# eliesgalvira/pragma-dsp

Measured on AMD Instinct MI355X. Metric: batched 1D FFT GSample/s at N=4096 batch=65536; achieved HBM GB/s vs peak, higher is better.
Workload: dtype f32

## Files before the change

### pragma-dsp_amd/csrc/pdsp_fft_kernel.h

```cpp
#pragma once

#include <hip/hip_runtime.h>

#include <type_traits>
#include <utility>

#include "pdsp_radix.h"

namespace pdsp {

#ifdef PDSP_STAMPS
__device__ unsigned long long pdsp_stamp_acc[64];
#define PDSP_STAMP_INIT() unsigned long long stamp_last_ = clock64()
#define PDSP_STAMP(slot)                                                          \
  do {                                                                            \
    __builtin_amdgcn_sched_barrier(0);                                            \
    const unsigned long long t_ = clock64();                                      \
    if (threadIdx.x == 0) atomicAdd(&pdsp_stamp_acc[slot], t_ - stamp_last_);     \
    stamp_last_ = clock64();                                                      \
    __builtin_amdgcn_sched_barrier(0);                                            \
  } while (0)
#else
#define PDSP_STAMP_INIT() ((void)0)
#define PDSP_STAMP(slot) ((void)0)
#endif

template <typename T> struct vec2;
template <> struct vec2<float> { using type = float2; };
template <> struct vec2<double> { using type = double2; };

template <typename T>
using cx = T __attribute__((ext_vector_type(2)));

template <int... Is, class F>
__device__ __forceinline__ void static_for_impl(std::integer_sequence<int, Is...>, F &&f) {
  (f(std::integral_constant<int, Is>{}), ...);
}
template <int N, class F>
__device__ __forceinline__ void static_for(F &&f) {
  static_for_impl(std::make_integer_sequence<int, N>{}, static_cast<F &&>(f));
}

constexpr int ilog2(int v) {
  int l = 0;
  while ((1 << l) < v) ++l;
  return l;
}
constexpr int bitrev(int x, int bits) {
  int y = 0;
  for (int b = 0; b < bits; ++b) {
    y = (y << 1) | (x & 1);
    x >>= 1;
  }
  return y;
}

template <typename T, int E, int I = 0>
__device__ __forceinline__ void pin_regs(T __attribute__((ext_vector_type(2))) (&a)[E]) {
  if constexpr (I < E) {
    asm volatile("" : "+v"(a[I]));
    pin_regs<T, E, I + 1>(a);
  }
}


template <typename T>
__device__ __forceinline__ cx<T> mul_neg_i(const cx<T> a) {
  return cx<T>{a.y, -a.x};
}
template <typename T>
__device__ __forceinline__ cx<T> conj(const cx<T> a) {
  return cx<T>{a.x, -a.y};
}
template <typename T>
__device__ __forceinline__ cx<T> add_mul_neg_i(const cx<T> a, const cx<T> b) {
  if constexpr (std::is_same_v<T, float>) {
    return __builtin_elementwise_fma(__builtin_shufflevector(b, b, 1, 0), cx<float>{1.0f, -1.0f}, a);
  } else {
    return cx<T>{a.x + b.y, a.y - b.x};
  }
}
template <typename T>
__device__ __forceinline__ cx<T> add_mul_pos_i(const cx<T> a, const cx<T> b) {
  if constexpr (std::is_same_v<T, float>) {
    return __builtin_elementwise_fma(__builtin_shufflevector(b, b, 1, 0), cx<float>{-1.0f, 1.0f}, a);
  } else {
    return cx<T>{a.x - b.y, a.y + b.x};
  }
}
template <typename T>
__device__ __forceinline__ cx<T> cmul(const cx<T> a, const cx<T> w) {
  if constexpr (std::is_same_v<T, float>) {
    cx<float> r;
    asm("v_pk_mul_f32 %0, %1, %2 op_sel:[0,0] op_sel_hi:[0,1]\n\t"
        "v_pk_fma_f32 %0, %1, %2, %0 op_sel:[1,1,0] op_sel_hi:[1,0,1] neg_lo:[0,1,0]"
        : "=&v"(r)
        : "v"(a), "v"(w));
    return r;
  } else {
    return a.xx * w + a.yy * cx<T>{-w.y, w.x};
  }
}

template <typename T, int M>
__device__ __forceinline__ cx<T> mul_w16(const cx<T> a) {
  constexpr T C1 = T(0.92387953251128673848);
  constexpr T C2 = T(0.70710678118654752440);
  constexpr T C3 = T(0.38268343236508977173);
  if constexpr (M == 0) {
    return a;
  } else if constexpr (M == 4) {
    return mul_neg_i(a);
  } else if constexpr (M == 2) {
    return add_mul_neg_i(a, a) * C2;
  } else if constexpr (M == 6) {
    return add_mul_pos_i(a, a) * (-C2);
  } else {
    constexpr T c = M == 1 ? C1 : M == 3 ? C3 : M == 5 ? -C3 : -C1;
    constexpr T s = M == 1 ? -C3 : M == 3 ? -C1 : M == 5 ? -C1 : -C3;
    return a.xx * cx<T>{c, s} + a.yy * cx<T>{-s, c};
  }
}

template <typename T, int NUM>
__device__ __forceinline__ cx<T> mul_w32(const cx<T> a);

template <typename T>
__device__ __forceinline__ void bfly4(cx<T> &a0, cx<T> &a1, cx<T> &a2, cx<T> &a3) {
  const cx<T> t0 = a0 + a2, t1 = a0 - a2, t2 = a1 + a3, t3 = a1 - a3;
  a0 = t0 + t2;
  a2 = t0 - t2;
  a1 = add_mul_neg_i(t1, t3);
  a3 = add_mul_pos_i(t1, t3);
}
template <typename T>
__device__ __forceinline__ void bfly4_x2_rot(cx<T> &a0, cx<T> &a1, cx<T> &d, cx<T> &a3) {
  const cx<T> t0 = add_mul_neg_i(a0, d), t1 = add_mul_pos_i(a0, d), t2 = a1 + a3, t3 = a1 - a3;
  a0 = t0 + t2;
  d = t0 - t2;
  a1 = add_mul_neg_i(t1, t3);
  a3 = add_mul_pos_i(t1, t3);
}

template <typename T, int R>
__device__ __forceinline__ void fft_reg(cx<T> (&a)[R]) {
  static_assert(R >= 1 && R <= 32 && (R & (R - 1)) == 0, "radix");
  if constexpr (R == 4) {
    bfly4(a[0], a[1], a[2], a[3]);
    const cx<T> x1 = a[1];
    a[1] = a[2];
    a[2] = x1;
    return;
  } else if constexpr (R == 8) {
    static_for<4>([&](auto kc) {
      constexpr int k = kc;
      const cx<T> u = a[k], v = a[k + 4];
      a[k] = u + v;
      if constexpr (k == 2) a[k + 4] = u - v;
      else a[k + 4] = mul_w32<T, 4 * k>(u - v);
    });
    bfly4(a[0], a[1], a[2], a[3]);
    bfly4_x2_rot(a[4], a[5], a[6], a[7]);
    cx<T> o[8];
    static_for<8>([&](auto kc) {
      constexpr int k = kc;
      o[bitrev(k, 3)] = a[(k & 1) * 4 + (k >> 1)];
    });
    static_for<8>([&](auto kc) { a[kc] = o[kc]; });
    return;
  } else if constexpr (R == 16) {
    static_for<4>([&](auto jc) {
      constexpr int j = jc;
      bfly4(a[j], a[j + 4], a[j + 8], a[j + 12]);
      if constexpr (j > 0) {
        a[j + 4] = mul_w32<T, 2 * j>(a[j + 4]);
        if constexpr (j != 2) a[j + 8] = mul_w32<T, (4 * j) % 32>(a[j + 8]);
        a[j + 12] = mul_w32<T, (6 * j) % 32>(a[j + 12]);
      }
    });
    bfly4(a[0], a[1], a[2], a[3]);
    bfly4(a[4], a[5], a[6], a[7]);
    bfly4_x2_rot(a[8], a[9], a[10], a[11]);
    bfly4(a[12], a[13], a[14], a[15]);
    cx<T> o[16];
    static_for<16>([&](auto kc) {
      constexpr int k = kc;
      o[bitrev(k, 4)] = a[4 * (k & 3) + (k >> 2)];
    });
    static_for<16>([&](auto kc) { a[kc] = o[kc]; });
    return;
  }
  static_for<ilog2(R)>([&](auto stc) {
    constexpr int s = R >> (stc + 1);
    static_for<R / 2>([&](auto ic) {
      constexpr int g = (ic / s) * 2 * s, k = ic % s;
      constexpr int i0 = g + k, i1 = i0 + s;
      const cx<T> u = a[i0], v = a[i1];
      a[i0] = u + v;
      a[i1] = mul_w32<T, k *(16 / s)>(u - v);
    });
  });
}

template <int LOG2N, int LOG2E = 4>
struct FftTraits {
  static constexpr RadixPlan P = make_radix_plan(LOG2N, LOG2E);
  static constexpr int N = P.n, E = P.e, TP = P.tp, NP = P.np;
  static constexpr int WG = TP >= 256 ? TP : 256;
  static constexpr int ROWS = WG / TP;
  static constexpr int LROW = N + N / 16;
  static constexpr int LDS_ELEMS = NP > 1 ? ROWS * LROW : 1;
};

template <int LOG2M>
constexpr int kPackedWG = FftTraits<LOG2M, packed_log2e(LOG2M)>::WG;

__device__ __forceinline__ int lds_pad(int i) { return i + (i >> 4); }
constexpr int cpad(int c) { return c + c / 16; }

template <int TP>
__device__ __forceinline__ long long uniform_row(long long row) {
  if constexpr (TP >= 64) return (long long)__builtin_amdgcn_readfirstlane((int)row);
  else return row;
}

__device__ __forceinline__ void load_order_fence() { __builtin_amdgcn_sched_barrier(0); }

template <typename T>
__device__ __forceinline__ T ld_stream(const T *p) { return __builtin_nontemporal_load(p); }
template <typename T>
__device__ __forceinline__ void st_stream(T v, T *p) { __builtin_nontemporal_store(v, p); }

__device__ __forceinline__ float mag(const cx<float> z) {
  const cx<float> s = z * z;
  return __builtin_amdgcn_sqrtf(s.x + s.y);
}
__device__ __forceinline__ double mag(const cx<double> z) { return hypot(z.x, z.y); }

template <typename T, bool THREE>
__device__ __forceinline__ void fused_window_pairs(const cx<T> c0, const cx<T> *__restrict__ we, const T k0, const T k1,
                                                   const T k2, cx<T> (&w)[4]) {
  static_for<4>([&](auto h) {
    const cx<T> e0 = we[2 * h], e1 = we[2 * h + 1];
    const cx<T> c = cx<T>{e0.x, e1.x} * c0.x - cx<T>{e0.y, e1.y} * c0.y;
    if constexpr (THREE) w[h] = c * (c * k2 + k1) + k0;
    else w[h] = c * k1 + k0;
  });
}


template <typename T>
struct LoadComplex {
  const T *__restrict__ re;
  const T *__restrict__ im;
  long long n;
  __device__ __forceinline__ cx<T> operator()(long long row, int off, int lane) const {
    const size_t o = (size_t)row * (size_t)n + (size_t)off;
    return cx<T>{ld_stream(re + o + (unsigned)lane), ld_stream(im + o + (unsigned)lane)};
  }
  static constexpr bool kPlanar = true;
  static constexpr bool kHasIm = true;
  static constexpr bool kPacked = false;
  __device__ __forceinline__ const T *plane_re() const { return re; }
  __device__ __forceinline__ const T *plane_im() const { return im; }
};

template <typename T>
struct LoadReal {
  const T *__restrict__ re;
  long long n;
  __device__ __forceinline__ cx<T> operator()(long long row, int off, int lane) const {
    return cx<T>{ld_stream(re + (size_t)row * (size_t)n + (size_t)off + (unsigned)lane), T(0)};
  }
  static constexpr bool kPlanar = true;
  static constexpr bool kHasIm = false;
  static constexpr bool kPacked = false;
  __device__ __forceinline__ const T *plane_re() const { return re; }
  __device__ __forceinline__ const T *plane_im() const { return nullptr; }
};

template <typename T, int WIN>
struct LoadPackedFrames {
  const T *__restrict__ x;
  const T *__restrict__ win;
  long long stride;
  const float *wb, *wq, *we;
  float k0, k1, k2;
  static constexpr bool kPlanar = true;
  static constexpr bool kHasIm = true;
  static constexpr bool kPacked = true;
  static constexpr int kWin = WIN;
};

template <typename T, bool CONJ>
struct LoadInterleaved {
  const cx<T> *__restrict__ z;
  long long n;
  __device__ __forceinline__ cx<T> operator()(long long row, int off, int lane) const {
    cx<T> v = ld_stream(z + (size_t)row * (size_t)n + (size_t)off + (unsigned)lane);
    if constexpr (CONJ) v.y = -v.y;
    return v;
  }
  static constexpr bool kPlanar = false;
  static constexpr bool kHasIm = true;
};

template <typename T, bool CONJ>
struct StoreInterleaved {
  cx<T> *__restrict__ z;
  long long n;
  T scale;
  __device__ __forceinline__ void operator()(long long row, int off, int lane, cx<T> v) const {
    v = v * scale;
    if constexpr (CONJ) v.y = -v.y;
    st_stream(v, z + (size_t)row * (size_t)n + (size_t)off + (unsigned)lane);
  }
  static constexpr bool kPlanar = false;
};

template <typename T, bool HAS_WIN>
struct LoadFrameWindowed {
  const T *__restrict__ x;
  const T *__restrict__ win;
  long long frame_len;
  long long stride;
  __device__ __forceinline__ cx<T> operator()(long long row, int off, int lane) const {
    const int i = off + lane;
    const int last = (int)frame_len - 1;
    T v = ld_stream(x + (size_t)row * (size_t)stride + (unsigned)(i < last ? i : last));
    v = i <= last ? v : T(0);
    if constexpr (HAS_WIN) v *= win[i];
    return cx<T>{v, T(0)};
  }
};

template <typename T>
struct StoreComplex {
  T *__restrict__ re;
  T *__restrict__ im;
  long long n;
  T scale;
  __device__ __forceinline__ void operator()(long long row, int off, int lane, cx<T> v) const {
    const size_t o = (size_t)row * (size_t)n + (size_t)off;
    v = v * scale;
    st_stream(v.x, re + o + (unsigned)lane);
    st_stream(v.y, im + o + (unsigned)lane);
  }
  static constexpr bool kPlanar = true;
};

template <typename T>
struct StoreAmplitude {
  T *__restrict__ amp;
  T *__restrict__ ph;
  int bins;
  int nyq;
  T s_edge;
  T s_mid;
  __device__ __forceinline__ void operator()(long long row, int off, int lane, cx<T> v) const {
    const int i = off + lane;
    if (i < bins) {
      const size_t o = (size_t)row * (size_t)bins;
      st_stream(mag(v) * ((i == 0 || i == nyq) ? s_edge : s_mid), amp + o + (unsigned)i);
      if (ph) st_stream(T(atan2(v.y, v.x)), ph + o + (unsigned)i);
    }
  }
};


template <typename T, int LOG2N, int LOG2E = 4>
struct TableTwiddles {
  const cx<T> *__restrict__ tw;
  template <int p, int r, int b>
  __device__ __forceinline__ cx<T> get(const int j) const {
    using TR = FftTraits<LOG2N, LOG2E>;
    constexpr int Ns = TR::P.ns[p];
    return (tw + (TR::P.twoff[p] + (r - 1) * Ns))[(unsigned)(j & (Ns - 1))];
  }
};

template <typename T, int NUM>
__device__ __forceinline__ cx<T> mul_w32(const cx<T> a) {
  constexpr int m = ((NUM % 32) + 32) % 32;
  if constexpr (m % 2 == 0) {
    constexpr int h = m / 2;
    if constexpr (h >= 8) return -mul_w16<T, h - 8>(a);
    else return mul_w16<T, h>(a);
  } else {
    constexpr double C[9] = {1.0, 0.98078528040323044913, 0.92387953251128675613, 0.83146961230254523708,
                             0.70710678118654752440, 0.55557023301960222474, 0.38268343236508977173,
                             0.19509032201612826785, 0.0};
    constexpr int q = m % 16;
    constexpr bool neg = m >= 16;
    constexpr int lo = q <= 8 ? q : 16 - q;
    constexpr double cq = q <= 8 ? C[lo] : -C[lo];
    constexpr double sq = C[8 - lo];
    constexpr T c = T(neg ? -cq : cq), s = T(neg ? sq : -sq);
    return a.xx * cx<T>{c, s} + a.yy * cx<T>{-s, c};
  }
}

template <typename T, int LOG2N, int LOG2E = 4>
struct RegTwiddles {
  using TR = FftTraits<LOG2N, LOG2E>;
  static_assert(LOG2E == 4, "the W16 correction of the short last pass assumes TP = N/16");
  static constexpr int nb(int p) { return TR::P.ns[p] > 1 ? (TR::P.r[p] == 16 ? 6 : TR::P.r[p] - 1) : 0; }
  static constexpr int off(int p) {
    int o = 0;
    for (int i = 0; i < p; ++i) o += nb(i);
    return o;
  }
  static constexpr int TOTAL = off(TR::NP) > 0 ? off(TR::NP) : 1;
  static constexpr int base_r(int R, int i) { return R == 16 ? (i < 4 ? i + 1 : (i - 2) * 4) : i + 1; }

  cx<T> tb[TOTAL];

  __device__ __forceinline__ void load(const cx<T> *__restrict__ tw, const int tid) {
    static_for<TR::NP>([&](auto pc) {
      constexpr int p = pc;
      constexpr int Ns = TR::P.ns[p], R = TR::P.r[p];
      if constexpr (Ns > 1) {
        const unsigned k0 = (unsigned)(Ns <= TR::TP ? (tid & (Ns - 1)) : tid);
        static_for<nb(p)>([&](auto ic) {
          constexpr int r = base_r(R, ic);
          tb[off(p) + ic] = (tw + (TR::P.twoff[p] + (r - 1) * Ns))[k0];
        });
      }
    });
  }

  template <int p, int r, int b>
  __device__ __forceinline__ cx<T> get(const int) const {
    constexpr int Ns = TR::P.ns[p], R = TR::P.r[p], O = off(p);
    cx<T> w;
    if constexpr (R == 16) {
      constexpr int hi = r & 12, lo = r & 3;
      if constexpr (hi == 0) w = tb[O + lo - 1];
      else if constexpr (lo == 0) w = tb[O + 2 + hi / 4];
      else w = cmul(tb[O + 2 + hi / 4], tb[O + lo - 1]);
    } else {
      w = tb[O + r - 1];
    }
    if constexpr (Ns > TR::TP && b > 0) w = mul_w32<T, 2 * ((r * b) % 16)>(w);
    return w;
  }
};


template <typename T, int LOG2N, bool LAST_TO_LDS, int LOG2E, int p, class TWF, int EE>
__device__ __forceinline__ void fft_pass_compute(cx<T> (&x)[EE], cx<T> *const lrow, const TWF &twf, const int tid) {
  using TR = FftTraits<LOG2N, LOG2E>;
  constexpr int E = TR::E, TP = TR::TP, NP = TR::NP;
  static_assert(EE == E, "register array size must be the plan's points per thread");
  constexpr bool kConstOffsets = (TP % 16 == 0);
  constexpr int R = TR::P.r[p], Ns = TR::P.ns[p], EB = E / R, LR = ilog2(R);
  constexpr bool last = (p == NP - 1);
  constexpr bool to_lds = !last || LAST_TO_LDS;

  static_for<EB>([&](auto bc) {
    constexpr int b = bc;
    cx<T> a[R];
    static_for<R>([&](auto rc) { a[rc] = x[b + rc * EB]; });
    const int j = tid + b * TP;
    if constexpr (Ns > 1) {
      static_for<R - 1>([&](auto rc) {
        constexpr int r = rc + 1;
        a[r] = cmul(a[r], twf.template get<p, r, b>(j));
      });
    }
    fft_reg<T, R>(a);
    if constexpr (!to_lds) {
      static_for<R>([&](auto rc) { x[b + rc * EB] = a[bitrev(rc, LR)]; });
    } else if constexpr (kConstOffsets) {
      constexpr int cb = Ns <= TP ? b * TP * R : b * TP;
      const int j0t = Ns <= TP ? ((tid >> ilog2(Ns)) << ilog2(Ns * R)) + (tid & (Ns - 1)) : tid;
      cx<T> *const wbase = lrow + lds_pad(j0t);
      static_for<R>([&](auto rc) { wbase[cpad(cb + rc * Ns)] = a[bitrev(rc, LR)]; });
    } else {
      const int j0 = ((j >> ilog2(Ns)) << ilog2(Ns * R)) + (j & (Ns - 1));
      static_for<R>([&](auto rc) { lrow[lds_pad(j0 + rc * Ns)] = a[bitrev(rc, LR)]; });
    }
  });
}

template <typename T, int LOG2N, int LOG2E, int EE>
__device__ __forceinline__ void fft_pass_readback(cx<T> (&x)[EE], const cx<T> *const lrow, const int tid) {
  using TR = FftTraits<LOG2N, LOG2E>;
  constexpr int E = TR::E, TP = TR::TP;
  if constexpr (TP % 16 == 0) {
    const cx<T> *const rbase = lrow + lds_pad(tid);
    static_for<E>([&](auto q) { x[q] = rbase[cpad(TP * q)]; });
  } else {
    static_for<E>([&](auto q) { x[q] = lrow[lds_pad(tid + TP * q)]; });
  }
}

template <typename T, int LOG2N, bool LAST_TO_LDS, int LOG2E = 4, class TWF = void, int EE = 0>
__device__ __forceinline__ void fft_passes(cx<T> (&x)[EE], cx<T> *const lrow, const TWF &twf, const int tid) {
  PDSP_STAMP_INIT();
  constexpr int NP = FftTraits<LOG2N, LOG2E>::NP;
  static_for<NP>([&](auto pc) {
    constexpr int p = pc;
    fft_pass_compute<T, LOG2N, LAST_TO_LDS, LOG2E, p>(x, lrow, twf, tid);
    PDSP_STAMP(8 + 4 * p);
    if constexpr (p != NP - 1) {
      __syncthreads();
      PDSP_STAMP(9 + 4 * p);
      fft_pass_readback<T, LOG2N, LOG2E>(x, lrow, tid);
      if constexpr (p + 1 < NP - 1 || LAST_TO_LDS) __syncthreads();
      PDSP_STAMP(10 + 4 * p);
    }
  });
}

struct PeakRec {
  int index;
  float frequency;
  float amplitude;
  float phase;
};

template <typename T>
struct PeakBest {
  T v;
  int i;
  cx<T> x;
  __device__ __forceinline__ void consider(const T ov, const int oi, const cx<T> ox) {
    if (ov > v || (ov == v && ov > T(0) && oi < i)) {
      v = ov;
      i = oi;
      x = ox;
    }
  }
  __device__ __forceinline__ void consider_ascending(const T ov, const int oi, const cx<T> ox) {
    if (ov > v) {
      v = ov;
      i = oi;
      x = ox;
    }
  }
  __device__ __forceinline__ void consider_descending(const T ov, const int oi, const cx<T> ox) {
    if (ov >= v) {
      v = ov;
      i = oi;
      x = ox;
    }
  }
};


template <typename T, int LOG2N, class LD, class ST>
__global__ void __launch_bounds__(FftTraits<LOG2N>::WG)
fft_stockham_kernel(const LD ld, const ST st, const typename vec2<T>::type *__restrict__ tw,
                    const long long batch) {
  using TR = FftTraits<LOG2N>;
  constexpr int E = TR::E, TP = TR::TP, NP = TR::NP;

  __shared__ cx<T> lds[TR::LDS_ELEMS];

  const int tid = TP == 1 ? 0 : (int)(threadIdx.x % TP);
  const int rloc = (int)(threadIdx.x / TP);
  const long long row_raw = (long long)blockIdx.x * TR::ROWS + rloc;
  const bool live = row_raw < batch;
  const long long row = uniform_row<TP>(live ? row_raw : batch - 1);
  cx<T> *const lrow = lds + (NP > 1 ? rloc * TR::LROW : 0);

  cx<T> x[E];
  constexpr bool kRegTw = (TP >= 16 && NP > 1);
  std::conditional_t<kRegTw, RegTwiddles<T, LOG2N>, TableTwiddles<T, LOG2N>> twf;
  static_for<E>([&](auto q) { x[q] = ld(row, TP * q, tid); });
  if constexpr (kRegTw) twf.load(reinterpret_cast<const cx<T> *>(tw), tid);
  if constexpr (!kRegTw) twf.tw = reinterpret_cast<const cx<T> *>(tw);
  fft_passes<T, LOG2N, false>(x, lrow, twf, tid);
  if (live) {
    static_for<E>([&](auto q) { st(row, TP * q, tid, x[q]); });
  }
}

template <typename T, int LOG2N, class LD, class ST>
__global__ void __launch_bounds__(256)
fft_staged_kernel(const LD ld, const ST st, const typename vec2<T>::type *__restrict__ tw, const long long batch) {
  using TR = FftTraits<LOG2N>;
  constexpr int N = TR::N, E = TR::E, TP = TR::TP, ROWS = TR::ROWS, WG = 256;
  static_assert(TR::WG == WG && TR::NP > 1 && N % 16 == 0, "staged path: 32 <= N <= 256");
  constexpr int CHUNK = ROWS * N;
  typedef T V4 __attribute__((ext_vector_type(4)));
  __shared__ cx<T> lds[TR::LDS_ELEMS];

  const int t = (int)threadIdx.x;
  const int tid = t % TP, rloc = t / TP;
  cx<T> *const lrow = lds + rloc * TR::LROW;
  const size_t base = (size_t)blockIdx.x * CHUNK;
  const size_t limit = (size_t)batch * N;
  const T *const pre = ld.plane_re();
  const T *const pim = ld.plane_im();

  static_for<CHUNK / 4 / WG>([&](auto ic) {
    const int p = 4 * (t + WG * ic);
    size_t g = base + (size_t)p;
    g = g + 4 <= limit ? g : limit - 4;
    const V4 r = ld_stream(reinterpret_cast<const V4 *>(pre + g));
    V4 m = V4{T(0), T(0), T(0), T(0)};
    if constexpr (LD::kHasIm) m = ld_stream(reinterpret_cast<const V4 *>(pim + g));
    cx<T> *const d = lds + (p / N) * TR::LROW + lds_pad(p % N);
    d[0] = cx<T>{r.x, m.x};
    d[1] = cx<T>{r.y, m.y};
    d[2] = cx<T>{r.z, m.z};
    d[3] = cx<T>{r.w, m.w};
  });
  __syncthreads();
  cx<T> x[E];
  {
    const cx<T> *const rbase = lrow + lds_pad(tid);
    static_for<E>([&](auto q) { x[q] = rbase[cpad(TP * q)]; });
  }
  __syncthreads();

  RegTwiddles<T, LOG2N> twf;
  twf.load(reinterpret_cast<const cx<T> *>(tw), tid);
  fft_passes<T, LOG2N, true>(x, lrow, twf, tid);
  __syncthreads();

  static_for<CHUNK / 4 / WG>([&](auto ic) {
    const int p = 4 * (t + WG * ic);
    const size_t g = base + (size_t)p;
    if (g + 4 <= limit) {
      const cx<T> *const d = lds + (p / N) * TR::LROW + lds_pad(p % N);
      const cx<T> v0 = d[0] * st.scale, v1 = d[1] * st.scale, v2 = d[2] * st.scale, v3 = d[3] * st.scale;
      st_stream(V4{v0.x, v1.x, v2.x, v3.x}, reinterpret_cast<V4 *>(st.re + g));
      st_stream(V4{v0.y, v1.y, v2.y, v3.y}, reinterpret_cast<V4 *>(st.im + g));
    }
  });
}

template <typename T, int LOG2N, bool AMP, class LD>
__global__ void __launch_bounds__(256)
fft_tiny_staged_kernel(const LD ld, const T *__restrict__ win, T *__restrict__ o1, T *__restrict__ o2, const T scale,
                       const int bins, const int nyq, const T s_edge, const T s_mid, const long long batch) {
  constexpr int N = 1 << LOG2N, WG = 256, CHUNK = 4096, ROWS = CHUNK / N, RPT = ROWS >= WG ? ROWS / WG : 1;
  static_assert(LOG2N >= 1 && LOG2N <= 5, "tiny path: 2 <= N <= 32 (N = 32: half the threads hold a row)");
  typedef T V4 __attribute__((ext_vector_type(4)));
  __shared__ cx<T> lds[CHUNK + CHUNK / 16];
  const int t = (int)threadIdx.x;
  const size_t base = (size_t)blockIdx.x * CHUNK;
  const size_t limit = (size_t)batch * N;
  const T *const pre = ld.plane_re();
  const T *const pim = ld.plane_im();

  static_for<CHUNK / 4 / WG>([&](auto ic) {
    const int p = 4 * (t + WG * ic);
    size_t g = base + (size_t)p;
    if (limit >= 4) g = g + 4 <= limit ? g : limit - 4;
    V4 r, m = V4{T(0), T(0), T(0), T(0)};
    if (limit >= 4) {
      r = ld_stream(reinterpret_cast<const V4 *>(pre + g));
      if constexpr (LD::kHasIm) m = ld_stream(reinterpret_cast<const V4 *>(pim + g));
    } else {
      r = V4{pre[0], pre[1], T(0), T(0)};
      if constexpr (LD::kHasIm) m = V4{pim[0], pim[1], T(0), T(0)};
    }
    if constexpr (N == 2) {
      const size_t g0 = base + (size_t)p;
      if (limit >= 4 && g0 < limit && g0 + 4 > limit) {
        r = V4{r.z, r.w, T(0), T(0)};
        m = V4{m.z, m.w, T(0), T(0)};
      }
    }
    cx<T> *const d = lds + lds_pad(p);
    d[0] = cx<T>{r.x, m.x};
    d[1] = cx<T>{r.y, m.y};
    d[2] = cx<T>{r.z, m.z};
    d[3] = cx<T>{r.w, m.w};
  });
  __syncthreads();

  cx<T> x[RPT][N];
  const bool holds_row = ROWS >= WG || t < ROWS;
  static_for<RPT>([&](auto rc) {
    const int row = holds_row ? t + WG * rc : ROWS - 1;
    static_for<N>([&](auto q) {
      cx<T> v = lds[lds_pad(row * N + q)];
      if constexpr (AMP) {
        if (win) v = v * win[q];
      }
      x[rc][q] = v;
    });
    fft_reg<T, N>(x[rc]);
  });
  __syncthreads();

  if constexpr (!AMP) {
    static_for<RPT>([&](auto rc) {
      const int row = t + WG * rc;
      if (holds_row) static_for<N>([&](auto k) { lds[lds_pad(row * N + k)] = x[rc][bitrev(k, LOG2N)] * scale; });
    });
    __syncthreads();
    static_for<CHUNK / 4 / WG>([&](auto ic) {
      const int p = 4 * (t + WG * ic);
      const size_t g = base + (size_t)p;
      const cx<T> *const d = lds + lds_pad(p);
      if (g + 4 <= limit) {
        st_stream(V4{d[0].x, d[1].x, d[2].x, d[3].x}, reinterpret_cast<V4 *>(o1 + g));
        st_stream(V4{d[0].y, d[1].y, d[2].y, d[3].y}, reinterpret_cast<V4 *>(o2 + g));
      } else if (g < limit) {
        for (int j = 0; j < 4 && g + j < limit; ++j) {
          o1[g + j] = d[j].x;
          o2[g + j] = d[j].y;
        }
      }
    });
  } else {
    T *const ampf = reinterpret_cast<T *>(lds);
    static_for<RPT>([&](auto rc) {
      const int row = t + WG * rc;
      static_for<N>([&](auto k) {
        if (holds_row && k < bins)
          ampf[row * bins + k] = mag(x[rc][bitrev(k, LOG2N)]) * ((k == 0 || k == nyq) ? s_edge : s_mid);
      });
    });
    __syncthreads();
    const size_t out_base = (size_t)blockIdx.x * ROWS * (size_t)bins, out_limit = (size_t)batch * (size_t)bins;
    const int out_count = ROWS * bins;
    for (int i = t; i < out_count; i += WG)
      if (out_base + (size_t)i < out_limit) o1[out_base + (size_t)i] = ampf[i];
  }
}

struct WinFused {
  const float *base;
  const float *step;
  float k0, k1, k2;
  float edge_ratio;
};

template <typename T, int LOG2M, bool FAST, int WIN, bool PEAK>
__global__ void __launch_bounds__(kPackedWG<LOG2M>)
spectrum_packed_kernel(const T *__restrict__ frames, const T *__restrict__ win, const WinFused wf, const long long frame_len,
                       const long long stride, const typename vec2<T>::type *__restrict__ tw,
                       const typename vec2<T>::type *__restrict__ twr, T *__restrict__ amp,
                       T *__restrict__ ph, const int two_sided, const T s_edge, const T s_mid,
                       PeakRec *__restrict__ peaks, const T freq_scale, const long long batch) {
  constexpr int LOG2E = packed_log2e(LOG2M);
  using TR = FftTraits<LOG2M, LOG2E>;
  constexpr int E = TR::E, TP = TR::TP, M = TR::N;
  static_assert(LOG2M >= 5, "packed path needs TP >= 2");
  constexpr bool HAS_WIN = WIN == 1;
  static_assert(WIN <= 1 || (FAST && sizeof(T) == 4 && LOG2E == 4), "fused windows: whole f32 frames");
  constexpr bool kAdj = FAST && LOG2E == 4 && TP >= 32;
  typedef T V4 __attribute__((ext_vector_type(4)));

  __shared__ cx<T> lds[TR::LDS_ELEMS];

  const int tid = (int)(threadIdx.x % TP);
  const int rloc = (int)(threadIdx.x / TP);
  const long long row_raw = (long long)blockIdx.x * TR::ROWS + rloc;
  const bool live = row_raw < batch;
  const long long row = uniform_row<TP>(live ? row_raw : batch - 1);
  cx<T> *const lrow = lds + rloc * TR::LROW;

  const T *const xrow = frames + (size_t)row * (size_t)stride;
  cx<T> x[E];
  constexpr bool kRegTw = (LOG2E == 4 && TP >= 16);
  std::conditional_t<kRegTw, RegTwiddles<T, LOG2M, LOG2E>, TableTwiddles<T, LOG2M, LOG2E>> twf;
  cx<T> twk0;
  V4 tb = V4{T(0), T(0), T(0), T(0)};
  V4 wb4 = V4{T(0), T(0), T(0), T(0)};
  cx<T> wv[HAS_WIN ? E : 1];
  if constexpr (kRegTw) twf.load(reinterpret_cast<const cx<T> *>(tw), tid);
  if constexpr (kAdj) tb = reinterpret_cast<const V4 *>(twr)[(unsigned)tid];
  else twk0 = reinterpret_cast<const cx<T> *>(twr)[(unsigned)tid];
  if constexpr (WIN >= 2) wb4 = reinterpret_cast<const V4 *>(wf.base)[(unsigned)tid];
  if constexpr (HAS_WIN && FAST) {
    const cx<T> *const w2 = reinterpret_cast<const cx<T> *>(win);
    static_for<E>([&](auto q) { wv[q] = (w2 + TP * q)[(unsigned)tid]; });
  } else if constexpr (HAS_WIN) {
    static_for<E>([&](auto q) { wv[q] = cx<T>{(win + 2 * TP * q)[2 * (unsigned)tid], (win + 2 * TP * q + 1)[2 * (unsigned)tid]}; });
  }
  load_order_fence();
  if constexpr (FAST) {
    const cx<T> *const x2 = reinterpret_cast<const cx<T> *>(xrow);
    static_for<E>([&](auto q) { x[q] = ld_stream(x2 + TP * q + (unsigned)tid); });
  } else {
    const int flen = (int)frame_len;
    static_for<E>([&](auto q) {
      const int i0 = 2 * (tid + TP * q);
      const int c0 = i0 < flen - 1 ? i0 : flen - 1, c1 = i0 + 1 < flen - 1 ? i0 + 1 : flen - 1;
      const T v0 = ld_stream(xrow + (unsigned)c0), v1 = ld_stream(xrow + (unsigned)c1);
      x[q] = cx<T>{i0 < flen ? v0 : T(0), i0 + 1 < flen ? v1 : T(0)};
    });
  }
  PDSP_STAMP_INIT();
  if constexpr (!kRegTw) twf.tw = reinterpret_cast<const cx<T> *>(tw);
  load_order_fence();
  if constexpr (HAS_WIN) static_for<E>([&](auto q) { x[q] = x[q] * wv[q]; });
  if constexpr (WIN >= 2) {
    static_assert(WIN < 2 || kAdj, "the fused windows' pre-scaled frames are split by the adjacent-bin code");
    const cx<T> cb{wb4.x, wb4.z}, sb{wb4.y, wb4.w};
    const T k0 = wf.k0, k1 = wf.k1, k2 = wf.k2;
    const cx<T> kc = cb * k1, ks = sb * k1;
    static_for<E>([&](auto qc) {
      constexpr int q = qc;
      const T cq = wf.step[2 * q], sq = wf.step[2 * q + 1];
      if constexpr (WIN == 3) {
        const cx<T> c = cb * cq - sb * sq;
        x[q] = x[q] * (k0 + c * (k1 + k2 * c));
      } else {
        x[q] = x[q] * ((k0 + kc * cq) - ks * sq);
      }
    });
  }
  const T edge = WIN >= 2 ? T(wf.edge_ratio) : s_edge / s_mid;
  if constexpr (kAdj && WIN <= 1) {
    const T g = T(0.5) * s_mid;
    static_for<E>([&](auto q) { x[q] = x[q] * g; });
  }
#ifdef PDSP_STAMPS
  pin_regs<T, E>(x);
#endif
  PDSP_STAMP(0);

  fft_passes<T, LOG2M, true, LOG2E>(x, lrow, twf, tid);
  __syncthreads();
  PDSP_STAMP(1);

  const int bins = (!FAST && two_sided) ? 2 * M : M + 1;
  const bool store_amp = live && (!PEAK || amp != nullptr);
  T *const arow = amp + (size_t)row * (size_t)bins;
  T *const prow = (!FAST && ph) ? ph + (size_t)row * (size_t)bins : nullptr;
  PeakBest<T> best{T(0), 0, cx<T>{T(0), T(0)}};
  T dc_amp = T(0);
  cx<T> dc_x{T(0), T(0)};
  if constexpr (kAdj) {
    typedef T V2 __attribute__((ext_vector_type(2)));
    const cx<T> tw0{tb.x, tb.y}, tw1{tb.z, tb.w};
    static_for<4>([&](auto qc) {
      constexpr int q = qc;
      const int k0 = 2 * (tid + TP * q);
      const cx<T> z0 = lrow[lds_pad(k0)], z1 = lrow[lds_pad(k0) + 1];
      const cx<T> zp0 = lrow[lds_pad((M - k0) & (M - 1))], zp1 = lrow[lds_pad(M - k0 - 1)];
      const cx<T> w0 = mul_w32<T, 2 * q>(tw0), w1 = mul_w32<T, 2 * q>(tw1);
      const cx<T> e0 = z0 + conj(zp0), p0 = cmul(z0 - conj(zp0), w0);
      const cx<T> e1 = z1 + conj(zp1), p1 = cmul(z1 - conj(zp1), w1);
      cx<T> xa0 = add_mul_neg_i(e0, p0), xb0 = conj(add_mul_pos_i(e0, p0));
      const cx<T> xa1 = add_mul_neg_i(e1, p1), xb1 = conj(add_mul_pos_i(e1, p1));
      if constexpr (q == 0) {
        const T r = tid == 0 ? edge : T(1);
        xa0 = xa0 * r;
        xb0 = xb0 * r;
      }
      const T ma0 = mag(xa0), mb0 = mag(xb0), ma1 = mag(xa1), mb1 = mag(xb1);
      if constexpr (PEAK) {
        if (k0 == 0) {
          dc_amp = ma0;
          dc_x = xa0;
        } else {
          best.consider(ma0, k0, xa0);
        }
        best.consider(ma1, k0 + 1, xa1);
        best.consider(mb1, M - k0 - 1, xb1);
        best.consider(mb0, M - k0, xb0);
      }
      if (store_amp) {
        __builtin_nontemporal_store(V2{ma0, ma1}, reinterpret_cast<V2 *>(arow + (unsigned)k0));
        __builtin_nontemporal_store(V2{mb1, mb0}, reinterpret_cast<V2 *>(arow + (unsigned)(M - k0 - 1)));
      }
    });
    if (tid == 0) {
      const cx<T> xm = conj(lrow[lds_pad(M / 2)]) * T(2);
      const T mm = mag(xm);
      if constexpr (PEAK) best.consider(mm, M / 2, xm);
      if (store_amp) arow[(unsigned)(M / 2)] = mm;
    }
  }
  const cx<T> *const zlo = lrow + lds_pad(tid);
  const cx<T> *const zhi = lrow + lds_pad(M - tid);
  const cx<T> *const zhi0 = lrow + lds_pad((M - tid) & (M - 1));
  static_for<kAdj ? 0 : E / 2 + 1>([&](auto qc) {
    constexpr int q = qc;
// ... 1455 lines not shown
```

Baseline: 415.1.

## Fold twiddles into radix-16 butterflies, use buffer loads, skip unit scaling

Result: no change. 415.9 (median of 3 runs) (+0.2%).

```diff
diff --git a/pragma-dsp_amd/csrc/pdsp_fft_kernel.h b/pragma-dsp_amd/csrc/pdsp_fft_kernel.h
--- a/pragma-dsp_amd/csrc/pdsp_fft_kernel.h
+++ b/pragma-dsp_amd/csrc/pdsp_fft_kernel.h
@@ -100,6 +100,25 @@
   } else {
     return a.xx * w + a.yy * cx<T>{-w.y, w.x};
   }
+}
+
+template <typename T>
+__device__ __forceinline__ cx<T> cmul_add(const cx<T> a, const cx<T> w, const cx<T> c) {
+  if constexpr (std::is_same_v<T, float>) {
+    cx<float> r;
+    asm("v_pk_fma_f32 %0, %1, %2, %3 op_sel:[0,0,0] op_sel_hi:[0,1,1]\n\t"
+        "v_pk_fma_f32 %0, %1, %2, %0 op_sel:[1,1,0] op_sel_hi:[1,0,1] neg_lo:[0,1,0]"
+        : "=&v"(r)
+        : "v"(a), "v"(w), "v"(c));
+    return r;
+  } else {
+    const cx<T> r = __builtin_elementwise_fma(a.xx, w, c);
+    return __builtin_elementwise_fma(a.yy, cx<T>{-w.y, w.x}, r);
+  }
+}
+template <typename T>
+__device__ __forceinline__ cx<T> twice_minus(const cx<T> a, const cx<T> s) {
+  return __builtin_elementwise_fma(a, cx<T>{T(2), T(2)}, -s);
 }
 
 template <typename T, int M>
@@ -133,6 +152,19 @@
   a1 = add_mul_neg_i(t1, t3);
   a3 = add_mul_pos_i(t1, t3);
 }
+template <typename T, bool TW0>
+__device__ __forceinline__ void bfly4_tw(cx<T> &x0, cx<T> &x1, cx<T> &x2, cx<T> &x3, const cx<T> w0, const cx<T> w1,
+                                         const cx<T> w2, const cx<T> w3) {
+  cx<T> A0 = x0;
+  if constexpr (TW0) A0 = cmul(x0, w0);
+  const cx<T> A1 = cmul(x1, w1);
+  const cx<T> t0 = cmul_add(x2, w2, A0), t1 = twice_minus(A0, t0);
+  const cx<T> t2 = cmul_add(x3, w3, A1), t3 = twice_minus(A1, t2);
+  x0 = t0 + t2;
+  x2 = t0 - t2;
+  x1 = add_mul_neg_i(t1, t3);
+  x3 = add_mul_pos_i(t1, t3);
+}
 template <typename T>
 __device__ __forceinline__ void bfly4_x2_rot(cx<T> &a0, cx<T> &a1, cx<T> &d, cx<T> &a3) {
   const cx<T> t0 = add_mul_neg_i(a0, d), t1 = add_mul_pos_i(a0, d), t2 = a1 + a3, t3 = a1 - a3;
@@ -140,6 +172,28 @@
   d = t0 - t2;
   a1 = add_mul_neg_i(t1, t3);
   a3 = add_mul_pos_i(t1, t3);
+}
+
+template <typename T, int j>
+__device__ __forceinline__ void fft_reg16_twist(cx<T> (&a)[16]) {
+  if constexpr (j > 0) {
+    a[j + 4] = mul_w32<T, 2 * j>(a[j + 4]);
+    if constexpr (j != 2) a[j + 8] = mul_w32<T, (4 * j) % 32>(a[j + 8]);
+    a[j + 12] = mul_w32<T, (6 * j) % 32>(a[j + 12]);
+  }
+}
+template <typename T>
+__device__ __forceinline__ void fft_reg16_stage_b(cx<T> (&a)[16]) {
+  bfly4(a[0], a[1], a[2], a[3]);
+  bfly4(a[4], a[5], a[6], a[7]);
+  bfly4_x2_rot(a[8], a[9], a[10], a[11]);
+  bfly4(a[12], a[13], a[14], a[15]);
+  cx<T> o[16];
+  static_for<16>([&](auto kc) {
+    constexpr int k = kc;
+    o[bitrev(k, 4)] = a[4 * (k & 3) + (k >> 2)];
+  });
+  static_for<16>([&](auto kc) { a[kc] = o[kc]; });
 }
 
 template <typename T, int R>
@@ -172,22 +226,9 @@
     static_for<4>([&](auto jc) {
       constexpr int j = jc;
       bfly4(a[j], a[j + 4], a[j + 8], a[j + 12]);
-      if constexpr (j > 0) {
-        a[j + 4] = mul_w32<T, 2 * j>(a[j + 4]);
-        if constexpr (j != 2) a[j + 8] = mul_w32<T, (4 * j) % 32>(a[j + 8]);
-        a[j + 12] = mul_w32<T, (6 * j) % 32>(a[j + 12]);
-      }
-    });
-    bfly4(a[0], a[1], a[2], a[3]);
-    bfly4(a[4], a[5], a[6], a[7]);
-    bfly4_x2_rot(a[8], a[9], a[10], a[11]);
-    bfly4(a[12], a[13], a[14], a[15]);
-    cx<T> o[16];
-    static_for<16>([&](auto kc) {
-      constexpr int k = kc;
-      o[bitrev(k, 4)] = a[4 * (k & 3) + (k >> 2)];
-    });
-    static_for<16>([&](auto kc) { a[kc] = o[kc]; });
+      fft_reg16_twist<T, j>(a);
+    });
+    fft_reg16_stage_b<T>(a);
     return;
   }
   static_for<ilog2(R)>([&](auto stc) {
@@ -230,6 +271,27 @@
 __device__ __forceinline__ T ld_stream(const T *p) { return __builtin_nontemporal_load(p); }
 template <typename T>
 __device__ __forceinline__ void st_stream(T v, T *p) { __builtin_nontemporal_store(v, p); }
+template <typename T>
+__device__ __forceinline__ __amdgpu_buffer_rsrc_t row_rsrc(const T *row_start, const long long n) {
+  return __builtin_amdgcn_make_buffer_rsrc(const_cast<T *>(row_start), 0, (int)n * (int)sizeof(T), 0x00020000);
+}
+template <typename T>
+__device__ __forceinline__ T ld_row(const __amdgpu_buffer_rsrc_t rs, const int off, const int lane) {
+  if constexpr (sizeof(T) == 4) {
+    return __builtin_bit_cast(T, __builtin_amdgcn_raw_buffer_load_b32(rs, lane * 4, off * 4, 2 ));
+  } else {
+    return __builtin_bit_cast(T, __builtin_amdgcn_raw_buffer_load_b64(rs, lane * 8, off * 8, 2));
+  }
+}
+template <typename T>
+__device__ __forceinline__ void st_row(const T v, const __amdgpu_buffer_rsrc_t rs, const int off, const int lane) {
+  if constexpr (sizeof(T) == 4) {
+    __builtin_amdgcn_raw_buffer_store_b32(__builtin_bit_cast(unsigned, v), rs, lane * 4, off * 4, 2 );
+  } else {
+    typedef unsigned U2 __attribute__((ext_vector_type(2)));
+    __builtin_amdgcn_raw_buffer_store_b64(__builtin_bit_cast(U2, v), rs, lane * 8, off * 8, 2);
+  }
+}
 
 __device__ __forceinline__ float mag(const cx<float> z) {
   const cx<float> s = z * z;
@@ -258,6 +320,17 @@
     const size_t o = (size_t)row * (size_t)n + (size_t)off;
     return cx<T>{ld_stream(re + o + (unsigned)lane), ld_stream(im + o + (unsigned)lane)};
   }
+  struct Rows {
+    __amdgpu_buffer_rsrc_t re, im;
+    __device__ __forceinline__ cx<T> operator()(int off, int lane) const {
+      return cx<T>{ld_row<T>(re, off, lane), ld_row<T>(im, off, lane)};
+    }
+  };
+  __device__ __forceinline__ Rows rows(long long row) const {
+    const size_t o = (size_t)row * (size_t)n;
+    return Rows{row_rsrc(re + o, n), row_rsrc(im + o, n)};
+  }
+  static constexpr bool kBufferRows = true;
   static constexpr bool kPlanar = true;
   static constexpr bool kHasIm = true;
   static constexpr bool kPacked = false;
@@ -272,6 +345,14 @@
   __device__ __forceinline__ cx<T> operator()(long long row, int off, int lane) const {
     return cx<T>{ld_stream(re + (size_t)row * (size_t)n + (size_t)off + (unsigned)lane), T(0)};
   }
+  struct Rows {
+    __amdgpu_buffer_rsrc_t re;
+    __device__ __forceinline__ cx<T> operator()(int off, int lane) const { return cx<T>{ld_row<T>(re, off, lane), T(0)}; }
+  };
+  __device__ __forceinline__ Rows rows(long long row) const {
+    return Rows{row_rsrc(re + (size_t)row * (size_t)n, n)};
+  }
+  static constexpr bool kBufferRows = true;
   static constexpr bool kPlanar = true;
   static constexpr bool kHasIm = false;
   static constexpr bool kPacked = false;
@@ -303,6 +384,7 @@
   }
   static constexpr bool kPlanar = false;
   static constexpr bool kHasIm = true;
+  static constexpr bool kBufferRows = false;
 };
 
 template <typename T, bool CONJ>
@@ -311,11 +393,15 @@
   long long n;
   T scale;
   __device__ __forceinline__ void operator()(long long row, int off, int lane, cx<T> v) const {
-    v = v * scale;
+    raw(row, off, lane, v * scale);
+  }
+  __device__ __forceinline__ void raw(long long row, int off, int lane, cx<T> v) const {
     if constexpr (CONJ) v.y = -v.y;
     st_stream(v, z + (size_t)row * (size_t)n + (size_t)off + (unsigned)lane);
   }
   static constexpr bool kPlanar = false;
+  static constexpr bool kBufferRows = false;
+  static constexpr bool kHasScale = true;
 };
 
 template <typename T, bool HAS_WIN>
@@ -332,6 +418,7 @@
     if constexpr (HAS_WIN) v *= win[i];
     return cx<T>{v, T(0)};
   }
+  static constexpr bool kBufferRows = false;
 };
 
 template <typename T>
@@ -341,12 +428,29 @@
   long long n;
   T scale;
   __device__ __forceinline__ void operator()(long long row, int off, int lane, cx<T> v) const {
+    raw(row, off, lane, v * scale);
+  }
+  __device__ __forceinline__ void raw(long long row, int off, int lane, const cx<T> v) const {
     const size_t o = (size_t)row * (size_t)n + (size_t)off;
-    v = v * scale;
     st_stream(v.x, re + o + (unsigned)lane);
     st_stream(v.y, im + o + (unsigned)lane);
   }
+  struct Rows {
+    __amdgpu_buffer_rsrc_t re, im;
+    T scale;
+    __device__ __forceinline__ void operator()(int off, int lane, const cx<T> v) const { raw(off, lane, v * scale); }
+    __device__ __forceinline__ void raw(int off, int lane, const cx<T> v) const {
+      st_row<T>(v.x, re, off, lane);
+      st_row<T>(v.y, im, off, lane);
+    }
+  };
+  __device__ __forceinline__ Rows rows(long long row) const {
+    const size_t o = (size_t)row * (size_t)n;
+    return Rows{row_rsrc(re + o, n), row_rsrc(im + o, n), scale};
+  }
   static constexpr bool kPlanar = true;
+  static constexpr bool kBufferRows = true;
+  static constexpr bool kHasScale = true;
 };
 
 template <typename T>
@@ -365,6 +469,8 @@
       if (ph) st_stream(T(atan2(v.y, v.x)), ph + o + (unsigned)i);
     }
   }
+  static constexpr bool kBufferRows = false;
+  static constexpr bool kHasScale = false;
 };
 
 
@@ -446,8 +552,21 @@
   }
 };
 
-
-template <typename T, int LOG2N, bool LAST_TO_LDS, int LOG2E, int p, class TWF, int EE>
+template <typename T, int p, int b, class TWF>
+__device__ __forceinline__ void fft_reg16_tw(cx<T> (&a)[16], const TWF &twf, const int j) {
+  static_for<4>([&](auto cc) {
+    constexpr int c = cc;
+    cx<T> w0 = cx<T>{T(1), T(0)};
+    if constexpr (c > 0) w0 = twf.template get<p, c, b>(j);
+    bfly4_tw<T, (c > 0)>(a[c], a[c + 4], a[c + 8], a[c + 12], w0, twf.template get<p, c + 4, b>(j),
+                         twf.template get<p, c + 8, b>(j), twf.template get<p, c + 12, b>(j));
+    fft_reg16_twist<T, c>(a);
+  });
+  fft_reg16_stage_b<T>(a);
+}
+
+
+template <typename T, int LOG2N, bool LAST_TO_LDS, int LOG2E, int p, bool FOLD, class TWF, int EE>
 __device__ __forceinline__ void fft_pass_compute(cx<T> (&x)[EE], cx<T> *const lrow, const TWF &twf, const int tid) {
   using TR = FftTraits<LOG2N, LOG2E>;
   constexpr int E = TR::E, TP = TR::TP, NP = TR::NP;
@@ -462,13 +581,17 @@
     cx<T> a[R];
     static_for<R>([&](auto rc) { a[rc] = x[b + rc * EB]; });
     const int j = tid + b * TP;
-    if constexpr (Ns > 1) {
-      static_for<R - 1>([&](auto rc) {
-        constexpr int r = rc + 1;
-        a[r] = cmul(a[r], twf.template get<p, r, b>(j));
-      });
-    }
-    fft_reg<T, R>(a);
+    if constexpr (FOLD && R == 16 && Ns > 1) {
+      fft_reg16_tw<T, p, b>(a, twf, j);
+    } else {
+      if constexpr (Ns > 1) {
+        static_for<R - 1>([&](auto rc) {
+          constexpr int r = rc + 1;
+          a[r] = cmul(a[r], twf.template get<p, r, b>(j));
+        });
+      }
+      fft_reg<T, R>(a);
+    }
     if constexpr (!to_lds) {
       static_for<R>([&](auto rc) { x[b + rc * EB] = a[bitrev(rc, LR)]; });
     } else if constexpr (kConstOffsets) {
@@ -495,13 +618,13 @@
   }
 }
 
-template <typename T, int LOG2N, bool LAST_TO_LDS, int LOG2E = 4, class TWF = void, int EE = 0>
+template <typename T, int LOG2N, bool LAST_TO_LDS, int LOG2E = 4, bool FOLD = false, class TWF = void, int EE = 0>
 __device__ __forceinline__ void fft_passes(cx<T> (&x)[EE], cx<T> *const lrow, const TWF &twf, const int tid) {
   PDSP_STAMP_INIT();
   constexpr int NP = FftTraits<LOG2N, LOG2E>::NP;
   static_for<NP>([&](auto pc) {
     constexpr int p = pc;
-    fft_pass_compute<T, LOG2N, LAST_TO_LDS, LOG2E, p>(x, lrow, twf, tid);
+    fft_pass_compute<T, LOG2N, LAST_TO_LDS, LOG2E, p, FOLD>(x, lrow, twf, tid);
     PDSP_STAMP(8 + 4 * p);
     if constexpr (p != NP - 1) {
       __syncthreads();
@@ -568,12 +691,37 @@
   cx<T> x[E];
   constexpr bool kRegTw = (TP >= 16 && NP > 1);
   std::conditional_t<kRegTw, RegTwiddles<T, LOG2N>, TableTwiddles<T, LOG2N>> twf;
-  static_for<E>([&](auto q) { x[q] = ld(row, TP * q, tid); });
+  constexpr bool kLdRows = TP >= 64 && LD::kBufferRows, kStRows = TP >= 64 && ST::kBufferRows;
+  if constexpr (kLdRows) {
+    const auto lr = ld.rows(row);
+    static_for<E>([&](auto q) { x[q] = lr(TP * q, tid); });
+  } else {
+    static_for<E>([&](auto q) { x[q] = ld(row, TP * q, tid); });
+  }
   if constexpr (kRegTw) twf.load(reinterpret_cast<const cx<T> *>(tw), tid);
   if constexpr (!kRegTw) twf.tw = reinterpret_cast<const cx<T> *>(tw);
-  fft_passes<T, LOG2N, false>(x, lrow, twf, tid);
+  fft_passes<T, LOG2N, false, 4, true>(x, lrow, twf, tid);
   if (live) {
-    static_for<E>([&](auto q) { st(row, TP * q, tid, x[q]); });
+    if constexpr (ST::kHasScale) {
+      auto store = [&](auto scaled) {
+        if constexpr (kStRows) {
+          const auto sr = st.rows(row);
+          static_for<E>([&](auto q) {
+            if constexpr (scaled) sr(TP * q, tid, x[q]);
+            else sr.raw(TP * q, tid, x[q]);
+          });
+        } else {
+          static_for<E>([&](auto q) {
+            if constexpr (scaled) st(row, TP * q, tid, x[q]);
+            else st.raw(row, TP * q, tid, x[q]);
+          });
+        }
+      };
+      if (st.scale == T(1)) store(std::false_type{});
+      else store(std::true_type{});
+    } else {
+      static_for<E>([&](auto q) { st(row, TP * q, tid, x[q]); });
+    }
   }
 }
 
```
